# leggedrobotics/qed-splatter

Hardware: NVIDIA B200
Metric: fwd+bwd RGB+depth Mpix/s (higher is better)
Workload: dtype f32

## Files before the change

### qed_splatter_b200/csrc/isect.cu

```cuda
#include <cub/device/device_radix_sort.cuh>

#include "common.cuh"
#include "radix.cuh"
#include "scan.cuh"

namespace qed {

__global__ void isect_count_kernel(int64_t CN, const float2* __restrict__ means2d, const int32_t* __restrict__ radii,
                                   float tile_size, int tile_w, int tile_h, int32_t* __restrict__ tiles) {
    int64_t i = (int64_t)blockIdx.x * blockDim.x + threadIdx.x;
    if (i >= CN) return;
    int r = radii[i];
    int cnt = 0;
    if (r > 0) {
        float2 m = means2d[i];
        TileBox tb = tile_box(m.x, m.y, r, tile_size, tile_w, tile_h);
        cnt = (tb.x1 - tb.x0) * (tb.y1 - tb.y0);
    }
    tiles[i] = cnt;
}

__global__ void isect_emit_kernel(int C, int N, const float2* __restrict__ means2d, const int32_t* __restrict__ radii,
                                  const float* __restrict__ depths, const int64_t* __restrict__ cum, float tile_size, int tile_w,
                                  int tile_h, int tile_n_bits, int64_t* __restrict__ isect_ids, int32_t* __restrict__ flatten_ids) {
// ... 168 lines not shown
    uint64_t* tmp_keys = reinterpret_cast<uint64_t*>(ws);
    int32_t* tmp_vals = reinterpret_cast<int32_t*>(ws + align_up((size_t)n * 8, 256));
    void* hist = ws + align_up((size_t)n * 8, 256) + align_up((size_t)n * 4, 256);
    return radix_sort_pairs<uint64_t>(n, nullptr, reinterpret_cast<const uint64_t*>(keys_in), vals_in, reinterpret_cast<uint64_t*>(keys_out),
                                      vals_out, tmp_keys, tmp_vals, hist, end_bit, stream);
}

namespace qed {

struct PrepareLayout {
    size_t scan_ws, scan_state, keys[3], vals[3], hist, cum2, total;
};

static PrepareLayout prepare_layout(int64_t CN) {
    PrepareLayout L;
    size_t o = 0;
    auto take = [&](size_t bytes) {
        size_t r = o;
        o += align_up(bytes, 256);
        return r;
    };
    L.scan_ws = take(scan_workspace_bytes(CN));
    L.scan_state = take(2 * kFlatScanStateBytes);
    for (int i = 0; i < 3; ++i) L.keys[i] = take((size_t)CN * 8);
    for (int i = 0; i < 3; ++i) L.vals[i] = take((size_t)CN * 4);
    L.hist = take(radix_hist_bytes(CN));
    L.cum2 = take((size_t)CN * 8);
    L.total = o;
    return L;
}

template <typename KeyT>
struct CompactVisibleSink {
    int N;
    const float* depths;
    KeyT* keys;
    int32_t* vals;
    __device__ __forceinline__ void operator()(int64_t idx, int32_t flag, int64_t inc) const {
        if (!flag) return;
        const uint32_t db = (uint32_t)__float_as_int(depths[idx]);
        keys[inc - 1] = sizeof(KeyT) == 8 ? (KeyT)(((uint64_t)(idx / N) << 32) | db) : (KeyT)db;
        vals[inc - 1] = (int32_t)idx;
    }
};

constexpr int kEmitThreads = 256;
constexpr int kEmitTile = 1024;

__global__ void emit_boundaries_kernel(int64_t n_vis, int64_t n_isects, const int64_t* __restrict__ counts_dev, int64_t* __restrict__ clamped,
                                       const int64_t* __restrict__ cum2, int32_t* __restrict__ first_j) {
    pdl_enter();
    const int64_t j = (int64_t)blockIdx.x * blockDim.x + threadIdx.x;
    if (counts_dev) {
        const int64_t real_vis = counts_dev[0], real_isects = counts_dev[1];
        n_vis = real_vis < n_vis ? real_vis : n_vis;
        n_isects = real_isects <= n_isects ? real_isects : 0;
        if (n_isects == 0) n_vis = 0;
    }
    if (j == 0) {
        clamped[0] = n_vis;
        clamped[1] = n_isects;
    }
    if (j >= n_vis) return;
    const int64_t start = j > 0 ? cum2[j - 1] : 0, end = cum2[j];
    for (int64_t b = (start + kEmitTile - 1) / kEmitTile; b * kEmitTile < end; ++b) first_j[b] = (int32_t)j;
}

__global__ void __launch_bounds__(kEmitThreads) emit_sorted_kernel(int64_t n_vis, int64_t n_isects, const int64_t* __restrict__ clamped, int N,
                                                                  const int32_t* __restrict__ sorted_vals,
                                                                  const int64_t* __restrict__ cum2, const int32_t* __restrict__ first_j,
                                                                  const float2* __restrict__ means2d, const int32_t* __restrict__ radii,
                                                                  float tile_size, int tile_w, int tile_h, int tile_n_bits,
                                                                  uint32_t* __restrict__ tkeys, int32_t* __restrict__ tvals) {
    __shared__ int16_t s_lo[kEmitTile + 1], s_hi[kEmitTile + 1];
    __shared__ int32_t s_k0[kEmitTile + 1], s_first[kEmitTile + 1], s_idx[kEmitTile + 1];
    __shared__ int16_t s_bw[kEmitTile + 1], s_large[kEmitTile + 1];
    __shared__ __align__(16) uint32_t s_okey[kEmitTile];
    __shared__ __align__(16) int32_t s_oval[kEmitTile];
    __shared__ int s_nlarge;
    __shared__ int s_wsum[kEmitThreads / 32];
    pdl_enter();
    const uint32_t vb = blockIdx.x;
    const int64_t e0 = (int64_t)vb * kEmitTile;
    if (clamped) {
        n_vis = clamped[0];
        n_isects = clamped[1];
        if (e0 >= n_isects) return;
    }
    const int64_t e1 = min(e0 + kEmitTile, n_isects);
    const int64_t j0 = first_j[vb];
    int64_t j1;
    if (e1 >= n_isects) {
        j1 = n_vis - 1;
    } else {
        const int64_t jn = first_j[vb + 1];
        j1 = (jn > 0 && cum2[jn - 1] == e1) ? jn - 1 : jn;
// ... 27 lines not shown
            s_oval[lo + t] = idx;
            if (++rx == bw) {
                rx = 0;
                ++ry;
            }
        }
    }
    const int lane = threadIdx.x & 31, warp = threadIdx.x >> 5;
    const int nlarge = s_nlarge;
    for (int i = warp; i < nlarge; i += kEmitThreads / 32) {
        const int g = s_large[i];
        const int lo = s_lo[g], n = s_hi[g] - lo, k0 = s_k0[g];
        const int bw = s_bw[g], idx = s_idx[g], first = s_first[g];
        const float inv_bw = 1.0f / (float)bw;
        for (int t = lane; t < n; t += 32) {
            const int k = k0 + t;
            const int ry = (int)(((float)k + 0.5f) * inv_bw);
            const int rx = k - ry * bw;
            s_okey[lo + t] = (uint32_t)(first + ry * tile_w + rx);
            s_oval[lo + t] = idx;
        }
    }
    __syncthreads();
    for (int t = threadIdx.x; t < (int)(e1 - e0); t += kEmitThreads) {
        tkeys[e0 + t] = s_okey[t];
        tvals[e0 + t] = s_oval[t];
    }
}

__global__ void __launch_bounds__(kEmitThreads) emit_exact_kernel(int64_t n_vis, int64_t n_isects, const int64_t* __restrict__ clamped, int N,
                                                                 const int32_t* __restrict__ sorted_vals, const int64_t* __restrict__ cum2,
                                                                 const int32_t* __restrict__ first_j, const float2* __restrict__ means2d,
                                                                 const int32_t* __restrict__ radii, const float4* __restrict__ geom, int height,
                                                                 float tile_size, int tile_w, int tile_h, int tile_n_bits,
                                                                 uint32_t* __restrict__ tkeys, int32_t* __restrict__ tvals) {
    __shared__ int16_t s_lo[kEmitTile + 1], s_hi[kEmitTile + 1], s_large[kEmitTile + 1];
    __shared__ int32_t s_k0[kEmitTile + 1], s_idx[kEmitTile + 1];
    __shared__ __align__(16) uint32_t s_okey[kEmitTile];
    __shared__ __align__(16) int32_t s_oval[kEmitTile];
    __shared__ int s_nlarge;
    pdl_enter();
    const uint32_t vb = blockIdx.x;
    const int64_t e0 = (int64_t)vb * kEmitTile;
    if (clamped) {
        n_vis = clamped[0];
        n_isects = clamped[1];
    }
    if (e0 >= n_isects) return;
    const int64_t e1 = min(e0 + kEmitTile, n_isects);
    const int64_t j0 = first_j[vb];
    int64_t j1;
    if (e1 >= n_isects) {
        j1 = n_vis - 1;
    } else {
        const int64_t jn = first_j[vb + 1];
        j1 = (jn > 0 && cum2[jn - 1] == e1) ? jn - 1 : jn;
    }
    const int G = (int)(j1 - j0) + 1;
// ... 56 lines not shown
        const uint32_t cam_bits = (uint32_t)(idx / N) << tile_n_bits;
        int base = 0;
        for (int r0 = tb.y0; r0 < tb.y1 && base < k0 + n; r0 += 32) {
            const int ty = r0 + lane;
            int c0 = 0, c1 = 0;
            if (ty < tb.y1) exact_row_span(ec, ty, height, tb.x0, tb.x1, c0, c1);
            const int w = c1 - c0;
            int inc = w;
#pragma unroll
            for (int o = 1; o < 32; o <<= 1) {
                const int v = __shfl_up_sync(0xffffffffu, inc, o);
                if (lane >= o) inc += v;
            }
            const int row_start = base + inc - w;
            const int a = max(row_start, k0), b = min(row_start + w, k0 + n);
            for (int q = a; q < b; ++q) {
                s_okey[lo + (q - k0)] = cam_bits | (uint32_t)(ty * tile_w + c0 + (q - row_start));
                s_oval[lo + (q - k0)] = idx;
            }
            base += __shfl_sync(0xffffffffu, inc, 31);
        }
    }
    __syncthreads();
    for (int t = threadIdx.x; t < (int)(e1 - e0); t += kEmitThreads) {
        tkeys[e0 + t] = s_okey[t];
        tvals[e0 + t] = s_oval[t];
    }
}

constexpr int kComposePer = 4;
__global__ void __launch_bounds__(256) compose_ids_ranges_kernel(int64_t n_host, const int64_t* __restrict__ n_dev, const uint32_t* __restrict__ tkeys,
                                                                 const int32_t* __restrict__ flat, const float* __restrict__ depths, int C, int n_tiles,
                                                                 int tile_n_bits, int64_t* __restrict__ isect_ids, int32_t* __restrict__ offsets) {
    pdl_enter();
    const int64_t i0 = ((int64_t)blockIdx.x * blockDim.x + threadIdx.x) * kComposePer;
    const int64_t n = n_dev ? *n_dev : n_host;
    if (n_dev && offsets && i0 == 0) {
        offsets[(int64_t)C * n_tiles] = (int32_t)n;
        if (n == 0)
            for (int64_t t = 0; t < (int64_t)C * n_tiles; ++t) offsets[t] = 0;
    }
    if (i0 >= n) return;
    uint32_t key[kComposePer];
    if (i0 + kComposePer <= n) {
        const uint4 k4 = *reinterpret_cast<const uint4*>(tkeys + i0);
        key[0] = k4.x, key[1] = k4.y, key[2] = k4.z, key[3] = k4.w;
    } else {
#pragma unroll
        for (int k = 0; k < kComposePer; ++k) key[k] = i0 + k < n ? tkeys[i0 + k] : 0u;
    }
    const uint32_t mask = (1u << tile_n_bits) - 1u;
    uint32_t kp = i0 > 0 ? tkeys[i0 - 1] : 0u;
#pragma unroll
    for (int k = 0; k < kComposePer; ++k) {
        const int64_t i = i0 + k;
        if (i >= n) break;
        if (isect_ids) {
            const uint32_t db = (uint32_t)__float_as_int(depths[flat[i]]);
            isect_ids[i] = (int64_t)(((uint64_t)key[k] << 32) | db);
        }
        if (offsets) {
            const int64_t cur = (int64_t)(key[k] >> tile_n_bits) * n_tiles + (key[k] & mask);
            if (i == 0) {
                for (int64_t t = 0; t <= cur; ++t) offsets[t] = 0;
            } else if (key[k] != kp) {
                const int64_t prev = (int64_t)(kp >> tile_n_bits) * n_tiles + (kp & mask);
                for (int64_t t = prev + 1; t <= cur; ++t) offsets[t] = (int32_t)i;
            }
            if (i == n - 1) {
                for (int64_t t = cur + 1; t < (int64_t)C * n_tiles; ++t) offsets[t] = (int32_t)n;
            }
        }
        kp = key[k];
    }
}

static int bit_length(int64_t v) {
    int b = 0;
    while (((int64_t)1 << b) <= v) ++b;
    return b;
}

}

extern "C" size_t qed_isect_prepare_workspace_bytes(int64_t CN) { return prepare_layout(CN > 0 ? CN : 1).total; }

extern "C" int qed_isect_prepare(int C, int N, const float* depths, const int32_t* tiles_per_gauss, void* workspace,
                                 size_t workspace_bytes, int64_t* counts_dev, int64_t* counts_host_pinned, qed_stream_t stream_) {
    cudaStream_t stream = (cudaStream_t)stream_;
    if (C < 0 || N < 0 || !counts_dev) return QED_ERR_BAD_ARG;
    const int64_t CN = (int64_t)C * N;
    if (CN == 0) {
        QED_CUDA_TRY(cudaMemsetAsync(counts_dev, 0, 16, stream));
    } else {
        if (CN > 0x7fffffffLL) return QED_ERR_UNSUPPORTED;
        if (!depths || !tiles_per_gauss || !workspace) return QED_ERR_BAD_ARG;
        const PrepareLayout L = prepare_layout(CN);
        if (workspace_bytes < L.total) return QED_ERR_WORKSPACE;
        char* ws = reinterpret_cast<char*>(workspace);
        int32_t* vals0 = reinterpret_cast<int32_t*>(ws + L.vals[0]);
        int32_t* vals1 = reinterpret_cast<int32_t*>(ws + L.vals[1]);
        int32_t* vals2 = reinterpret_cast<int32_t*>(ws + L.vals[2]);
        int64_t* cum2 = reinterpret_cast<int64_t*>(ws + L.cum2);
        int rc;
        char* st0 = ws + L.scan_state;
        char* st1 = st0 + kFlatScanStateBytes;
        const bool flat = g_flat_scan != 0;
        if (flat) QED_CUDA_TRY(cudaMemsetAsync(st0, 0, 2 * kFlatScanStateBytes, stream));
        if (C == 1) {
            uint32_t* k0 = reinterpret_cast<uint32_t*>(ws + L.keys[0]);
            uint32_t* k1 = reinterpret_cast<uint32_t*>(ws + L.keys[1]);
            uint32_t* k2 = reinterpret_cast<uint32_t*>(ws + L.keys[2]);
            rc = flat ? scan_flat_to(CN, nullptr, ScanFlagPositive{tiles_per_gauss}, CompactVisibleSink<uint32_t>{N, depths, k0, vals0}, counts_dev, st0, stream)
                      : scan_inclusive_to(CN, nullptr, ScanFlagPositive{tiles_per_gauss}, CompactVisibleSink<uint32_t>{N, depths, k0, vals0}, counts_dev,
                                          ws + L.scan_ws, stream);
            if (rc != QED_OK) return rc;
            rc = radix_sort_pairs<uint32_t>(CN, counts_dev, k0, vals0, k1, vals1, k2, vals2, ws + L.hist, 32, stream);
        } else {
            uint64_t* k0 = reinterpret_cast<uint64_t*>(ws + L.keys[0]);
            uint64_t* k1 = reinterpret_cast<uint64_t*>(ws + L.keys[1]);
            uint64_t* k2 = reinterpret_cast<uint64_t*>(ws + L.keys[2]);
            rc = flat ? scan_flat_to(CN, nullptr, ScanFlagPositive{tiles_per_gauss}, CompactVisibleSink<uint64_t>{N, depths, k0, vals0}, counts_dev, st0, stream)
                      : scan_inclusive_to(CN, nullptr, ScanFlagPositive{tiles_per_gauss}, CompactVisibleSink<uint64_t>{N, depths, k0, vals0}, counts_dev,
                                          ws + L.scan_ws, stream);
            if (rc != QED_OK) return rc;
            rc = radix_sort_pairs<uint64_t>(CN, counts_dev, k0, vals0, k1, vals1, k2, vals2, ws + L.hist, 32 + bit_length(C - 1), stream);
        }
        if (rc != QED_OK) return rc;
        rc = flat ? scan_flat_to(CN, counts_dev, ScanGather{tiles_per_gauss, vals1}, ScanStore{cum2}, counts_dev + 1, st1, stream)
                  : scan_inclusive(CN, counts_dev, ScanGather{tiles_per_gauss, vals1}, cum2, counts_dev + 1, ws + L.scan_ws, stream);
        if (rc != QED_OK) return rc;
    }
    if (counts_host_pinned) QED_CUDA_TRY(cudaMemcpyAsync(counts_host_pinned, counts_dev, 16, cudaMemcpyDeviceToHost, stream));
    return QED_OK;
}

extern "C" size_t qed_isect_fill_workspace_bytes(int64_t n_isects) {
    if (n_isects <= 0) return 256;
    const size_t nb = (size_t)((n_isects + kEmitTile - 1) / kEmitTile + 1);
    return 5 * align_up((size_t)n_isects * 4, 256) + radix_hist_bytes(n_isects) + align_up(nb * 4, 256) + align_up(nb * 8 + 8, 256) + 256;
}

extern "C" int qed_isect_fill(int C, int N, int64_t n_visible, int64_t n_isects, const float* means2d, const int32_t* radii,
                              const float* depths, const float* geom, int image_width, int image_height, int tile_size, int tile_width,
                              int tile_height, const void* prepare_workspace, void* workspace, size_t workspace_bytes,
                              const int64_t* counts_dev, int64_t* isect_ids, int32_t* flatten_ids, int32_t* isect_offsets,
                              int64_t* n_exact_dev, qed_stream_t stream_) {
    cudaStream_t stream = (cudaStream_t)stream_;
    if (C < 0 || N < 0 || n_visible < 0 || n_isects < 0 || tile_size <= 0) return QED_ERR_BAD_ARG;
// ... 13 lines not shown
    if (n_isects > 0x7fffffffLL) return QED_ERR_UNSUPPORTED;
    if (n_exact_dev && !exact && !counts_dev && !isect_offsets) return QED_ERR_BAD_ARG;
    if (!means2d || !radii || !depths || !prepare_workspace || !workspace || !flatten_ids) return QED_ERR_BAD_ARG;
    if (workspace_bytes < qed_isect_fill_workspace_bytes(n_isects)) return QED_ERR_WORKSPACE;
    const int tile_n_bits = bit_length(n_tiles);
    const int cam_bits = bit_length(C - 1);
    if (tile_n_bits + cam_bits > 32) return QED_ERR_UNSUPPORTED;
    const PrepareLayout L = prepare_layout(CN);
    const char* pws = reinterpret_cast<const char*>(prepare_workspace);
    const int32_t* sorted_vals = reinterpret_cast<const int32_t*>(pws + L.vals[1]);
    const int64_t* cum2 = reinterpret_cast<const int64_t*>(pws + L.cum2);
    char* ws = reinterpret_cast<char*>(workspace);
    const size_t seg = align_up((size_t)n_isects * 4, 256);
    uint32_t* k0 = reinterpret_cast<uint32_t*>(ws);
    uint32_t* k1 = reinterpret_cast<uint32_t*>(ws + seg);
    uint32_t* k2 = reinterpret_cast<uint32_t*>(ws + 2 * seg);
    int32_t* v0 = reinterpret_cast<int32_t*>(ws + 3 * seg);
    int32_t* v2 = reinterpret_cast<int32_t*>(ws + 4 * seg);
    void* hist = ws + 5 * seg;
    const size_t nb = (size_t)((n_isects + kEmitTile - 1) / kEmitTile);
    int32_t* first_j = reinterpret_cast<int32_t*>(ws + 5 * seg + radix_hist_bytes(n_isects));
    int64_t* clamped = reinterpret_cast<int64_t*>(ws + 5 * seg + radix_hist_bytes(n_isects) + align_up((nb + 1) * 4, 256));
    if (n_visible == 0) return QED_ERR_BAD_ARG;
    QED_CUDA_TRY(launch_pdl(emit_boundaries_kernel, dim3((unsigned)((n_visible + 255) / 256)), dim3(256), 0, stream, n_visible, n_isects, counts_dev,
                            clamped, cum2, first_j));
    const int64_t* cl = counts_dev ? clamped : nullptr;
    if (exact) {
        QED_CUDA_TRY(launch_pdl(emit_exact_kernel, dim3((unsigned)nb), dim3(kEmitThreads), 0, stream, n_visible, n_isects, cl, N, sorted_vals, cum2,
                                first_j, reinterpret_cast<const float2*>(means2d), radii, reinterpret_cast<const float4*>(geom), image_height,
                                (float)tile_size, tile_width, tile_height, tile_n_bits, k0, v0));
    } else {
        QED_CUDA_TRY(launch_pdl(emit_sorted_kernel, dim3((unsigned)nb), dim3(kEmitThreads), 0, stream, n_visible, n_isects, cl, N, sorted_vals, cum2,
                                first_j, reinterpret_cast<const float2*>(means2d), radii, (float)tile_size, tile_width, tile_height, tile_n_bits,
                                k0, v0));
    }
    const int64_t* n_dev = has_end ? clamped + 1 : nullptr;
    int rc = radix_sort_pairs<uint32_t>(n_isects, n_dev, k0, v0, k1, flatten_ids, k2, v2, hist, tile_n_bits + cam_bits, stream);
    if (rc != QED_OK) return rc;
    QED_CUDA_TRY(launch_pdl(compose_ids_ranges_kernel, dim3((unsigned)((n_isects + 256 * kComposePer - 1) / (256 * kComposePer))), dim3(256), 0, stream,
                            n_isects, n_dev, k1, flatten_ids, depths, C, n_tiles, tile_n_bits, isect_ids, isect_offsets));
    if (n_exact_dev) QED_CUDA_TRY(cudaMemcpyAsync(n_exact_dev, clamped + 1, 8, cudaMemcpyDeviceToDevice, stream));
    return QED_OK;
}
```

### qed_splatter_b200/csrc/radix.cuh

```cuda
#pragma once
#include "common.cuh"

namespace qed {

static thread_local int g_radix_small_tiles = 0;
static thread_local int g_radix_onesweep = 1;

constexpr int kSortThreads = 256;
constexpr int kSortItems = 16;
constexpr int kSortTile = kSortThreads * kSortItems;
constexpr int kRadix = 256;

struct SegCounts {
    const int32_t* counts = nullptr;
    int shift = 0;
    __device__ __forceinline__ bool ok(int64_t i) const { return !counts || (int)(i & ((1 << shift) - 1)) < counts[i >> shift]; }
};

template <typename KeyT, bool SEG>
__global__ void __launch_bounds__(kSortThreads) radix_upsweep_kernel(int64_t n_host, const int64_t* n_dev, const KeyT* __restrict__ keys, int shift,
                                                                    uint32_t mask, int nblocks, uint32_t* __restrict__ hist , SegCounts seg) {
    __shared__ uint32_t sh[kRadix];
    pdl_enter();
    const int64_t n = n_dev ? *n_dev : n_host;
// ... 393 lines not shown
        global_base[d] = (sscan[8 + warp] + ginc - tot) + excl;
    }
    __syncthreads();
#pragma unroll
    for (int r = 0; r < kRounds; ++r) {
        const int local = warp * kPerWarp + r * 32 + lane;
        if (local < tile_n) {
            const uint32_t d = (uint32_t)(key[r] >> shift) & mask;
            const uint32_t pos = digit_start[d] + warp_hist[warp][d] + rank[r];
            skeys[pos] = key[r];
            svals[pos] = val[r];
        }
    }
    __syncthreads();
    for (int i = threadIdx.x; i < tile_n; i += kSortThreads) {
        const KeyT k = skeys[i];
        const uint32_t d = (uint32_t)(k >> shift) & mask;
        const int64_t dst = (int64_t)global_base[d] + (i - digit_start[d]);
        keys_out[dst] = k;
        vals_out[dst] = svals[i];
    }
}

inline size_t radix_hist_bytes(int64_t capacity) {
    int64_t nb = (capacity + kSortTile - 1) / kSortTile;
    if (nb < 1) nb = 1;
    return 2 * (((size_t)kRadix * nb * 4 + 255) / 256 * 256) + ((kRadix * 4 + 255) / 256 * 256) +
           (((size_t)kRadix * 2 * nb * 8 + 255) / 256 * 256) + ((size_t)(kMaxPasses * kRadix + kMaxPasses) * 4 + 255) / 256 * 256;
}

template <typename KeyT>
inline int radix_sort_pairs(int64_t capacity, const int64_t* n_dev, const KeyT* keys_in, const int32_t* vals_in, KeyT* keys_out,
                            int32_t* vals_out, KeyT* tmp_keys, int32_t* tmp_vals, void* hist_ws, int end_bit, cudaStream_t stream,
                            SegCounts seg = SegCounts()) {
    if (capacity <= 0) return QED_OK;
    const int nb = (int)((capacity + kSortTile - 1) / kSortTile);
    const size_t hist_bytes = ((size_t)kRadix * nb * 4 + 255) / 256 * 256;
    uint32_t* hist_a = reinterpret_cast<uint32_t*>(hist_ws);
    uint32_t* hist_b = reinterpret_cast<uint32_t*>(reinterpret_cast<char*>(hist_ws) + hist_bytes);
    uint32_t* totals = reinterpret_cast<uint32_t*>(reinterpret_cast<char*>(hist_ws) + 2 * hist_bytes);
    const int passes = (end_bit + 7) / 8;
    if (passes == 0) {
        if (n_dev) return QED_ERR_UNSUPPORTED;
        QED_CUDA_TRY(cudaMemcpyAsync(keys_out, keys_in, (size_t)capacity * sizeof(KeyT), cudaMemcpyDeviceToDevice, stream));
        QED_CUDA_TRY(cudaMemcpyAsync(vals_out, vals_in, (size_t)capacity * 4, cudaMemcpyDeviceToDevice, stream));
        return QED_OK;
    }
    if (!seg.counts && g_radix_onesweep && passes <= kMaxPasses && (nb <= kOnesweepMaxBlocks || g_radix_onesweep > 1)) {
        char* ows = reinterpret_cast<char*>(hist_ws) + 2 * hist_bytes + ((kRadix * 4 + 255) / 256 * 256);
        const bool small = g_radix_small_tiles && nb <= 2 * 148;
        const int nbk = small ? (int)((capacity + kSortTile / 2 - 1) / (kSortTile / 2)) : nb;
        uint64_t* status = reinterpret_cast<uint64_t*>(ows);
        const size_t status_bytes = ((size_t)kRadix * 2 * nb * 8 + 255) / 256 * 256;
        uint32_t* hist_all = reinterpret_cast<uint32_t*>(ows + status_bytes);
        uint32_t* tickets = hist_all + kMaxPasses * kRadix;
        QED_CUDA_TRY(cudaMemsetAsync(ows, 0, status_bytes + (size_t)(kMaxPasses * kRadix + kMaxPasses) * 4, stream));
        QED_CUDA_TRY(launch_pdl(radix_histogram_kernel<KeyT>, dim3(nb), dim3(kSortThreads), 0, stream, capacity, n_dev, keys_in, passes, end_bit, hist_all));
        auto one = small ? radix_onesweep_kernel<KeyT, 8> : radix_onesweep_kernel<KeyT, 16>;
        const size_t one_smem = small ? RadixSmem<KeyT>::kBytes - (size_t)(kSortTile / 2) * (sizeof(KeyT) + 4) : RadixSmem<KeyT>::kBytes;
        QED_CUDA_TRY(cudaFuncSetAttribute(one, cudaFuncAttributeMaxDynamicSharedMemorySize, (int)one_smem));
        const KeyT* sk = keys_in;
        const int32_t* sv = vals_in;
        for (int pass = 0; pass < passes; ++pass) {
            const bool to_out = ((passes - 1 - pass) % 2) == 0;
            KeyT* dk = to_out ? keys_out : tmp_keys;
            int32_t* dv = to_out ? vals_out : tmp_vals;
            const int bits = (end_bit - pass * 8) < 8 ? (end_bit - pass * 8) : 8;
            QED_CUDA_TRY(launch_pdl(one, dim3(nbk), dim3(kSortThreads), one_smem, stream, capacity, n_dev, sk, sv, dk, dv, pass * 8,
                                    (1u << bits) - 1u, pass, hist_all, status, tickets));
            sk = dk;
            sv = dv;
        }
        return QED_OK;
    }
    auto down = radix_downsweep_kernel<KeyT, false>;
    auto down_seg = radix_downsweep_kernel<KeyT, true>;
    QED_CUDA_TRY(cudaFuncSetAttribute(down, cudaFuncAttributeMaxDynamicSharedMemorySize, (int)RadixSmem<KeyT>::kBytes));
    if (seg.counts) QED_CUDA_TRY(cudaFuncSetAttribute(down_seg, cudaFuncAttributeMaxDynamicSharedMemorySize, (int)RadixSmem<KeyT>::kBytes));
    auto pass_mask = [&](int pass) {
        const int bits = (end_bit - pass * 8) < 8 ? (end_bit - pass * 8) : 8;
// ... 30 lines not shown
```

### qed_splatter_b200/csrc/scan.cuh

```cuda
#pragma once
#include "common.cuh"

namespace qed {

constexpr int kScanThreads = 256;
constexpr int kScanItems = 8;
constexpr int kScanTile = kScanThreads * kScanItems;

__device__ __forceinline__ int64_t block_exclusive_scan(int64_t v, int64_t* smem_warp, int64_t& total) {
    const int lane = threadIdx.x & 31, warp = threadIdx.x >> 5;
    int64_t inc = v;
#pragma unroll
    for (int o = 1; o < 32; o <<= 1) {
        int64_t t = __shfl_up_sync(0xffffffffu, inc, o);
        if (lane >= o) inc += t;
    }
    if (lane == 31) smem_warp[warp] = inc;
    __syncthreads();
    if (warp == 0) {
        int64_t w = lane < (kScanThreads / 32) ? smem_warp[lane] : 0;
        int64_t winc = w;
#pragma unroll
        for (int o = 1; o < 32; o <<= 1) {
            int64_t t = __shfl_up_sync(0xffffffffu, winc, o);
// ... 89 lines not shown
inline size_t scan_workspace_bytes(int64_t capacity) {
    int64_t nb = (capacity + kScanTile - 1) / kScanTile;
    return (size_t)(nb > 0 ? nb : 1) * sizeof(int64_t);
}

template <typename F, typename Sink>
inline int scan_inclusive_to(int64_t capacity, const int64_t* n_dev, F f, Sink sink, int64_t* total_dev, void* workspace, cudaStream_t stream) {
    int64_t nb = (capacity + kScanTile - 1) / kScanTile;
    if (nb == 0) nb = 1;
    int64_t* sums = reinterpret_cast<int64_t*>(workspace);
    QED_CUDA_TRY(launch_pdl(scan_reduce_kernel<F>, dim3((unsigned)nb), dim3(kScanThreads), 0, stream, capacity, n_dev, f, sums));
    QED_CUDA_TRY(launch_pdl(scan_sums_kernel, dim3(1), dim3(kScanThreads), 0, stream, nb, sums, total_dev));
    QED_CUDA_TRY(launch_pdl(scan_final_kernel<F, Sink>, dim3((unsigned)nb), dim3(kScanThreads), 0, stream, capacity, n_dev, f, sums, sink));
    return QED_OK;
}

constexpr int kFlatScanBlocks = 1024;
struct FlatScanState {
    unsigned long long agg[kFlatScanBlocks];
    unsigned int ticket, pad;
};
constexpr size_t kFlatScanStateBytes = sizeof(FlatScanState);

template <typename F, typename Sink>
__global__ void __launch_bounds__(kScanThreads) scan_flat_kernel(int64_t n_host, const int64_t* n_dev, F f, Sink sink, FlatScanState* __restrict__ st,
                                                                int64_t* __restrict__ total_dev, int tiles_per_block) {
    __shared__ int64_t sw[kScanThreads / 32 + 1];
    __shared__ unsigned int s_vb;
    pdl_enter();
    const int64_t n = n_dev ? min(*n_dev, n_host) : n_host;
    if (threadIdx.x == 0) s_vb = atomicAdd(&st->ticket, 1u);
    __syncthreads();
    const unsigned int vb = s_vb;
    const int64_t tile0 = (int64_t)vb * tiles_per_block;
    int32_t v[kScanItems];
    int64_t s = 0, ex0 = 0, total;
    if (tiles_per_block == 1) {
        const int64_t base = tile0 * kScanTile + (int64_t)threadIdx.x * kScanItems;
#pragma unroll
        for (int k = 0; k < kScanItems; ++k) {
            v[k] = (base + k < n) ? f(base + k) : 0;
            s += v[k];
        }
        ex0 = block_exclusive_scan(s, sw, total);
    } else {
        for (int t = 0; t < tiles_per_block; ++t) {
            const int64_t base = (tile0 + t) * kScanTile;
            if (base >= n) break;
#pragma unroll
            for (int k = 0; k < kScanItems; ++k) {
                const int64_t i = base + k * kScanThreads + threadIdx.x;
// ... 6 lines not shown
        volatile unsigned long long* slot = st->agg + vb;
        *slot = (1ull << 63) | (unsigned long long)total;
    }
    int64_t mine = 0;
    for (unsigned int b = threadIdx.x; b < vb; b += kScanThreads) {
        volatile const unsigned long long* slot = st->agg + b;
        unsigned long long w;
        do {
            w = *slot;
        } while (!(w >> 63));
        mine += (int64_t)(w & ~(1ull << 63));
    }
    int64_t prefix;
    block_exclusive_scan(mine, sw, prefix);
    if (vb == gridDim.x - 1 && threadIdx.x == 0 && total_dev) *total_dev = prefix + total;
    if (tiles_per_block == 1) {
        const int64_t base = tile0 * kScanTile + (int64_t)threadIdx.x * kScanItems;
        int64_t ex = ex0 + prefix;
#pragma unroll
        for (int k = 0; k < kScanItems; ++k) {
            ex += v[k];
            if (base + k < n) sink(base + k, v[k], ex);
        }
        return;
    }
    int64_t carry = prefix;
    for (int t = 0; t < tiles_per_block; ++t) {
        const int64_t tbase = (tile0 + t) * kScanTile;
        if (tbase >= n) break;
        const int64_t base = tbase + (int64_t)threadIdx.x * kScanItems;
        int64_t ts = 0;
#pragma unroll
        for (int k = 0; k < kScanItems; ++k) {
            v[k] = (base + k < n) ? f(base + k) : 0;
            ts += v[k];
        }
        int64_t tile_total;
        int64_t ex = block_exclusive_scan(ts, sw, tile_total) + carry;
#pragma unroll
        for (int k = 0; k < kScanItems; ++k) {
            ex += v[k];
            if (base + k < n) sink(base + k, v[k], ex);
        }
        carry += tile_total;
    }
}

template <typename F, typename Sink>
inline int scan_flat_to(int64_t capacity, const int64_t* n_dev, F f, Sink sink, int64_t* total_dev, void* state, cudaStream_t stream) {
    int64_t tiles = (capacity + kScanTile - 1) / kScanTile;
    if (tiles == 0) tiles = 1;
    const int blocks = (int)(tiles < kFlatScanBlocks ? tiles : kFlatScanBlocks);
    const int tiles_per_block = (int)((tiles + blocks - 1) / blocks);
    const int used = (int)((tiles + tiles_per_block - 1) / tiles_per_block);
    QED_CUDA_TRY(launch_pdl(scan_flat_kernel<F, Sink>, dim3((unsigned)used), dim3(kScanThreads), 0, stream, capacity, n_dev, f, sink,
                            reinterpret_cast<FlatScanState*>(state), total_dev, tiles_per_block));
    return QED_OK;
}

template <typename F>
inline int scan_inclusive(int64_t capacity, const int64_t* n_dev, F f, int64_t* out, int64_t* total_dev, void* workspace, cudaStream_t stream) {
    return scan_inclusive_to(capacity, n_dev, f, ScanStore{out}, total_dev, workspace, stream);
}

}
```

### qed_splatter_b200/pipeline.py

```python
from __future__ import annotations

from dataclasses import dataclass
from typing import Dict, Optional

import torch
from torch import Tensor

from . import _lib, ops
from ._lib import check, current_stream, ptr


@dataclass
class StepOutput:
    loss: Tensor
    grads: Dict[str, Tensor]
    packed_grads: Tensor
    radii: Tensor
    render: Tensor
    alphas: Tensor
    n_isects: int
    n_visible: Optional[int] = None
    v_viewmats: Optional[Tensor] = None


# ... 318 lines not shown
        def redo():
            self.overflow_repeats += 1
            return forward_and_loss(True)[2:]

        render, alphas, v_render, v_alphas = forward_and_loss(False)
        v_viewmats = self._get("v_viewmats", (C, 4, 4)) if pose_gradients else None
        grads, packed = self.backward(v_render, v_alphas, grad_out, n_chunks=n_chunks, on_chunk=on_chunk, exchange=exchange, v_viewmats=v_viewmats,
                                      _redo=redo)
        self._last_v = (v_render, v_alphas)
        f = self._fwd
        return StepOutput(loss=self._loss, grads=grads, packed_grads=packed, radii=f["radii"], render=f["render"], alphas=f["alphas"],
                          n_isects=f.get("n_isects_real", f["M"]), n_visible=f.get("n_visible"), v_viewmats=v_viewmats)

    def n_isects_exact(self) -> int:
        f = self._fwd
        return int(self._n_exact.item()) if (f.get("exact") and f["M"]) else int(f.get("n_isects_real", f["M"]))

    @property
    def launches_per_step(self) -> int:
        f = self._fwd
        tile_bits = (f["tw"] * f["th"]).bit_length()
        cam_bits = (f["C"] - 1).bit_length()

        def radix(capacity: int, bits: int, segmented: bool = False) -> int:
            passes = (bits + 7) // 8
            one_kernel_passes = (not segmented) and (capacity + 4095) // 4096 <= 444
            return 1 + passes if one_kernel_passes else 3 * passes

        if self.sort_impl == "two_level":
            isect = 1 + radix(f["C"] * f["N"], 32 + cam_bits) + 1 + 1 + 1 + radix(f["M"], tile_bits + cam_bits) + 1
        else:
            end_bit = 32 + tile_bits + f["C"].bit_length()
            isect = 3 + 1 + (radix(f["M"], end_bit) if self.sort_impl == "own" else 8) + 1
        return 1 + isect + 1 + 3 + 1 + 1

    @torch.no_grad()
    def count_pairs(self, which=("fwd", "bwd")) -> Dict[str, int]:
        lib, stream, f = self.lib, current_stream(), self._fwd
        out = {}
        if not f["M"]:
            return out
        names = ("entries_loaded", "entries_staged", "warp_candidates", "pairs_evaluated", "pairs_contributing", "reduction_groups")
        for which in which:
            cnt = torch.zeros(6, dtype=torch.int64, device=self.device)
            check(lib.qed_debug_set_raster_counters(ptr(cnt)), "set counters")
            try:
                if which == "fwd":
                    check(lib.qed_raster_fwd(f["C"], f["N"], f["M"], f["D"], ptr(f["geom"]), ptr(f["colors"]), ptr(f["backgrounds"]),
                                             f["width"], f["height"], 16, f["tw"], f["th"], ptr(f["offsets"]), int(f["has_end"]), ptr(f["flat"]),
                                             f["normalize"], ptr(f["render"]), ptr(f["alphas"]), ptr(f["last_ids"]), stream), "qed_raster_fwd(stats)")
                else:
                    v_render, v_alphas = self._last_v
                    scratch = torch.zeros(f["C"] * f["N"], 12, device=self.device)
                    check(lib.qed_raster_bwd(f["C"], f["N"], f["M"], f["D"], ptr(f["geom"]), ptr(f["colors"]), ptr(f["backgrounds"]),
                                             f["width"], f["height"], 16, f["tw"], f["th"], ptr(f["offsets"]), ptr(f["flat"]), f["normalize"],
                                             ptr(f["render"]), ptr(f["alphas"]), ptr(f["last_ids"]), ptr(v_render), ptr(v_alphas),
# ... 8 lines not shown
```

Measured before the change: 1741.

## Fuse radix histograms into producer kernels and compute tile offsets by counting

The visibility compaction scan now builds the per-pass radix digit histograms in shared memory, so the onesweep sort can skip its separate histogram kernel. The emit kernels atomically count intersections per tile bin, and a new single-block scan kernel turns those counts into tile offsets while also producing the second sort's histograms. This replaces the offset-writing logic in compose and drops the compose launch when isect ids are not requested. The memsets are merged and the workspace is reordered. In exchange it adds global and shared atomics and a serial single-block scan over all bins.

```diff
diff --git a/qed_splatter_b200/csrc/isect.cu b/qed_splatter_b200/csrc/isect.cu
--- a/qed_splatter_b200/csrc/isect.cu
+++ b/qed_splatter_b200/csrc/isect.cu
@@ -214,9 +214,9 @@
     };
     L.scan_ws = take(scan_workspace_bytes(CN));
     L.scan_state = take(2 * kFlatScanStateBytes);
+    L.hist = take(radix_hist_bytes(CN));
     for (int i = 0; i < 3; ++i) L.keys[i] = take((size_t)CN * 8);
     for (int i = 0; i < 3; ++i) L.vals[i] = take((size_t)CN * 4);
-    L.hist = take(radix_hist_bytes(CN));
     L.cum2 = take((size_t)CN * 8);
     L.total = o;
     return L;
@@ -224,15 +224,46 @@
 
 template <typename KeyT>
 struct CompactVisibleSink {
+    static constexpr int kPasses = sizeof(KeyT) == 8 ? kMaxPasses : 4;
     int N;
     const float* depths;
     KeyT* keys;
     int32_t* vals;
+    uint32_t* hist_all;
+    int end_bit;
+    __device__ static uint32_t* smem_hist() {
+        __shared__ uint32_t h[kPasses * kRadix];
+        return h;
+    }
+    __device__ __forceinline__ int passes() const { return (end_bit + 7) / 8; }
+    __device__ __forceinline__ void block_begin() const {
+        if (!hist_all) return;
+        for (int i = threadIdx.x; i < passes() * kRadix; i += blockDim.x) smem_hist()[i] = 0;
+        __syncthreads();
+    }
+    __device__ __forceinline__ void block_end() const {
+        if (!hist_all) return;
+        __syncthreads();
+        for (int i = threadIdx.x; i < passes() * kRadix; i += blockDim.x) {
+            const uint32_t c = smem_hist()[i];
+            if (c) atomicAdd(hist_all + i, c);
+        }
+    }
     __device__ __forceinline__ void operator()(int64_t idx, int32_t flag, int64_t inc) const {
         if (!flag) return;
         const uint32_t db = (uint32_t)__float_as_int(depths[idx]);
-        keys[inc - 1] = sizeof(KeyT) == 8 ? (KeyT)(((uint64_t)(idx / N) << 32) | db) : (KeyT)db;
+        const KeyT key = sizeof(KeyT) == 8 ? (KeyT)(((uint64_t)(idx / N) << 32) | db) : (KeyT)db;
+        keys[inc - 1] = key;
         vals[inc - 1] = (int32_t)idx;
+        if (hist_all) {
+            uint32_t* h = smem_hist();
+#pragma unroll
+            for (int p = 0; p < kPasses; ++p) {
+                if (p * 8 >= end_bit) break;
+                const int bits = end_bit - p * 8 < 8 ? end_bit - p * 8 : 8;
+                atomicAdd(&h[p * kRadix + ((uint32_t)(key >> (p * 8)) & ((1u << bits) - 1u))], 1u);
+            }
+        }
     }
 };
 
@@ -240,9 +271,12 @@
 constexpr int kEmitTile = 1024;
 
 __global__ void emit_boundaries_kernel(int64_t n_vis, int64_t n_isects, const int64_t* __restrict__ counts_dev, int64_t* __restrict__ clamped,
-                                       const int64_t* __restrict__ cum2, int32_t* __restrict__ first_j) {
+                                       const int64_t* __restrict__ cum2, int32_t* __restrict__ first_j, int32_t* __restrict__ bin_counts,
+                                       int64_t n_bins) {
     pdl_enter();
     const int64_t j = (int64_t)blockIdx.x * blockDim.x + threadIdx.x;
+    if (bin_counts)
+        for (int64_t t = j; t < n_bins; t += (int64_t)gridDim.x * blockDim.x) bin_counts[t] = 0;
     if (counts_dev) {
         const int64_t real_vis = counts_dev[0], real_isects = counts_dev[1];
         n_vis = real_vis < n_vis ? real_vis : n_vis;
@@ -258,12 +292,23 @@
     for (int64_t b = (start + kEmitTile - 1) / kEmitTile; b * kEmitTile < end; ++b) first_j[b] = (int32_t)j;
 }
 
+__device__ __forceinline__ void emit_store(int64_t e0, int n, const uint32_t* s_okey, const int32_t* s_oval, uint32_t* __restrict__ tkeys,
+                                           int32_t* __restrict__ tvals, int32_t* __restrict__ bin_counts, int n_tiles, int tile_n_bits) {
+    for (int t = threadIdx.x; t < n; t += kEmitThreads) {
+        const uint32_t key = s_okey[t];
+        tkeys[e0 + t] = key;
+        tvals[e0 + t] = s_oval[t];
+        if (bin_counts) atomicAdd(bin_counts + (key >> tile_n_bits) * (uint32_t)n_tiles + (key & ((1u << tile_n_bits) - 1u)), 1);
+    }
+}
+
 __global__ void __launch_bounds__(kEmitThreads) emit_sorted_kernel(int64_t n_vis, int64_t n_isects, const int64_t* __restrict__ clamped, int N,
                                                                   const int32_t* __restrict__ sorted_vals,
                                                                   const int64_t* __restrict__ cum2, const int32_t* __restrict__ first_j,
                                                                   const float2* __restrict__ means2d, const int32_t* __restrict__ radii,
                                                                   float tile_size, int tile_w, int tile_h, int tile_n_bits,
-                                                                  uint32_t* __restrict__ tkeys, int32_t* __restrict__ tvals) {
+                                                                  uint32_t* __restrict__ tkeys, int32_t* __restrict__ tvals,
+                                                                  int32_t* __restrict__ bin_counts) {
     __shared__ int16_t s_lo[kEmitTile + 1], s_hi[kEmitTile + 1];
     __shared__ int32_t s_k0[kEmitTile + 1], s_first[kEmitTile + 1], s_idx[kEmitTile + 1];
     __shared__ int16_t s_bw[kEmitTile + 1], s_large[kEmitTile + 1];
@@ -337,10 +382,7 @@
         }
     }
     __syncthreads();
-    for (int t = threadIdx.x; t < (int)(e1 - e0); t += kEmitThreads) {
-        tkeys[e0 + t] = s_okey[t];
-        tvals[e0 + t] = s_oval[t];
-    }
+    emit_store(e0, (int)(e1 - e0), s_okey, s_oval, tkeys, tvals, bin_counts, tile_w * tile_h, tile_n_bits);
 }
 
 __global__ void __launch_bounds__(kEmitThreads) emit_exact_kernel(int64_t n_vis, int64_t n_isects, const int64_t* __restrict__ clamped, int N,
@@ -348,7 +390,8 @@
                                                                  const int32_t* __restrict__ first_j, const float2* __restrict__ means2d,
                                                                  const int32_t* __restrict__ radii, const float4* __restrict__ geom, int height,
                                                                  float tile_size, int tile_w, int tile_h, int tile_n_bits,
-                                                                 uint32_t* __restrict__ tkeys, int32_t* __restrict__ tvals) {
+                                                                 uint32_t* __restrict__ tkeys, int32_t* __restrict__ tvals,
+                                                                 int32_t* __restrict__ bin_counts) {
     __shared__ int16_t s_lo[kEmitTile + 1], s_hi[kEmitTile + 1], s_large[kEmitTile + 1];
     __shared__ int32_t s_k0[kEmitTile + 1], s_idx[kEmitTile + 1];
     __shared__ __align__(16) uint32_t s_okey[kEmitTile];
@@ -451,24 +494,88 @@
         }
     }
     __syncthreads();
-    for (int t = threadIdx.x; t < (int)(e1 - e0); t += kEmitThreads) {
-        tkeys[e0 + t] = s_okey[t];
-        tvals[e0 + t] = s_oval[t];
+    emit_store(e0, (int)(e1 - e0), s_okey, s_oval, tkeys, tvals, bin_counts, tile_w * tile_h, tile_n_bits);
+}
+
+constexpr int kTileOffsetsThreads = 1024;
+constexpr int kTileOffsetsItems = 8;
+__global__ void __launch_bounds__(kTileOffsetsThreads) tile_offsets_kernel(int32_t* __restrict__ offsets, int64_t n_bins, int has_end, int n_tiles,
+                                                                          int tile_n_bits, int end_bit, uint32_t* __restrict__ hist_all,
+                                                                          int64_t* __restrict__ n_exact_dev) {
+    constexpr int kWarps = kTileOffsetsThreads / 32;
+    __shared__ uint32_t s_hist[4][kRadix];
+    __shared__ int64_t s_warp[kWarps];
+    __shared__ int64_t s_carry;
+    const int lane = threadIdx.x & 31, warp = threadIdx.x >> 5;
+    const int passes = (end_bit + 7) / 8;
+    if (hist_all)
+        for (int i = threadIdx.x; i < 4 * kRadix; i += kTileOffsetsThreads) (&s_hist[0][0])[i] = 0;
+    if (threadIdx.x == 0) s_carry = 0;
+    pdl_enter();
+    __syncthreads();
+    for (int64_t base = 0; base < n_bins; base += kTileOffsetsThreads * kTileOffsetsItems) {
+        const int64_t b0 = base + (int64_t)threadIdx.x * kTileOffsetsItems;
+        int32_t v[kTileOffsetsItems];
+        int64_t sum = 0;
+#pragma unroll
+        for (int k = 0; k < kTileOffsetsItems; ++k) {
+            v[k] = b0 + k < n_bins ? offsets[b0 + k] : 0;
+            sum += v[k];
+            if (hist_all && v[k]) {
+                const int64_t bin = b0 + k;
+                const uint32_t key = ((uint32_t)(bin / n_tiles) << tile_n_bits) | (uint32_t)(bin % n_tiles);
+                for (int p = 0; p < passes; ++p) {
+                    const int bits = end_bit - p * 8 < 8 ? end_bit - p * 8 : 8;
+                    atomicAdd(&s_hist[p][(key >> (p * 8)) & ((1u << bits) - 1u)], (uint32_t)v[k]);
+                }
+            }
+        }
+        int64_t inc = sum;
+#pragma unroll
+        for (int o = 1; o < 32; o <<= 1) {
+            const int64_t t = __shfl_up_sync(0xffffffffu, inc, o);
+            if (lane >= o) inc += t;
+        }
+        if (lane == 31) s_warp[warp] = inc;
+        __syncthreads();
+        if (warp == 0) {
+            const int64_t w = s_warp[lane];
+            int64_t winc = w;
+#pragma unroll
+            for (int o = 1; o < 32; o <<= 1) {
+                const int64_t t = __shfl_up_sync(0xffffffffu, winc, o);
+                if (lane >= o) winc += t;
+            }
+            s_warp[lane] = winc - w;
+        }
+        __syncthreads();
+        int64_t run = s_carry + s_warp[warp] + inc - sum;
+#pragma unroll
+        for (int k = 0; k < kTileOffsetsItems; ++k) {
+            if (b0 + k < n_bins) offsets[b0 + k] = (int32_t)run;
+            run += v[k];
+        }
+        __syncthreads();
+        if (threadIdx.x == kTileOffsetsThreads - 1) s_carry = run;
+        __syncthreads();
+    }
+    if (threadIdx.x == 0) {
+        if (has_end) offsets[n_bins] = (int32_t)s_carry;
+        if (n_exact_dev) *n_exact_dev = s_carry;
+    }
+    if (hist_all) {
+        __syncthreads();
+        for (int i = threadIdx.x; i < passes * kRadix; i += kTileOffsetsThreads) hist_all[i] = (&s_hist[0][0])[i];
     }
 }
 
 constexpr int kComposePer = 4;
-__global__ void __launch_bounds__(256) compose_ids_ranges_kernel(int64_t n_host, const int64_t* __restrict__ n_dev, const uint32_t* __restrict__ tkeys,
-                                                                 const int32_t* __restrict__ flat, const float* __restrict__ depths, int C, int n_tiles,
-                                                                 int tile_n_bits, int64_t* __restrict__ isect_ids, int32_t* __restrict__ offsets) {
+__global__ void __launch_bounds__(256) compose_ids_kernel(int64_t n_host, const int64_t* __restrict__ n_dev, const uint32_t* __restrict__ tkeys,
+                                                          const int32_t* __restrict__ flat, const float* __restrict__ depths,
+                                                          int64_t* __restrict__ isect_ids) {
     pdl_enter();
     const int64_t i0 = ((int64_t)blockIdx.x * blockDim.x + threadIdx.x) * kComposePer;
     const int64_t n = n_dev ? *n_dev : n_host;
-    if (n_dev && offsets && i0 == 0) {
-        offsets[(int64_t)C * n_tiles] = (int32_t)n;
-        if (n == 0)
-            for (int64_t t = 0; t < (int64_t)C * n_tiles; ++t) offsets[t] = 0;
-    }
     if (i0 >= n) return;
     uint32_t key[kComposePer];
     if (i0 + kComposePer <= n) {
@@ -478,29 +585,12 @@
 #pragma unroll
         for (int k = 0; k < kComposePer; ++k) key[k] = i0 + k < n ? tkeys[i0 + k] : 0u;
     }
-    const uint32_t mask = (1u << tile_n_bits) - 1u;
-    uint32_t kp = i0 > 0 ? tkeys[i0 - 1] : 0u;
 #pragma unroll
     for (int k = 0; k < kComposePer; ++k) {
         const int64_t i = i0 + k;
         if (i >= n) break;
-        if (isect_ids) {
-            const uint32_t db = (uint32_t)__float_as_int(depths[flat[i]]);
-            isect_ids[i] = (int64_t)(((uint64_t)key[k] << 32) | db);
-        }
-        if (offsets) {
-            const int64_t cur = (int64_t)(key[k] >> tile_n_bits) * n_tiles + (key[k] & mask);
-            if (i == 0) {
-                for (int64_t t = 0; t <= cur; ++t) offsets[t] = 0;
-            } else if (key[k] != kp) {
-                const int64_t prev = (int64_t)(kp >> tile_n_bits) * n_tiles + (kp & mask);
-                for (int64_t t = prev + 1; t <= cur; ++t) offsets[t] = (int32_t)i;
-            }
-            if (i == n - 1) {
-                for (int64_t t = cur + 1; t < (int64_t)C * n_tiles; ++t) offsets[t] = (int32_t)n;
-            }
-        }
-        kp = key[k];
+        const uint32_t db = (uint32_t)__float_as_int(depths[flat[i]]);
+        isect_ids[i] = (int64_t)(((uint64_t)key[k] << 32) | db);
     }
 }
 
@@ -535,25 +625,28 @@
         char* st0 = ws + L.scan_state;
         char* st1 = st0 + kFlatScanStateBytes;
         const bool flat = g_flat_scan != 0;
-        if (flat) QED_CUDA_TRY(cudaMemsetAsync(st0, 0, 2 * kFlatScanStateBytes, stream));
+        const int end_bit = C == 1 ? 32 : 32 + bit_length(C - 1);
+        const bool lookback = radix_lookback(CN, end_bit);
+        QED_CUDA_TRY(cudaMemsetAsync(st0, 0, (L.hist - L.scan_state) + (lookback ? radix_lookback_bytes(CN) : 0), stream));
+        uint32_t* hist_all = flat && lookback ? radix_hist_all(ws + L.hist, CN) : nullptr;
         if (C == 1) {
             uint32_t* k0 = reinterpret_cast<uint32_t*>(ws + L.keys[0]);
             uint32_t* k1 = reinterpret_cast<uint32_t*>(ws + L.keys[1]);
             uint32_t* k2 = reinterpret_cast<uint32_t*>(ws + L.keys[2]);
-            rc = flat ? scan_flat_to(CN, nullptr, ScanFlagPositive{tiles_per_gauss}, CompactVisibleSink<uint32_t>{N, depths, k0, vals0}, counts_dev, st0, stream)
-                      : scan_inclusive_to(CN, nullptr, ScanFlagPositive{tiles_per_gauss}, CompactVisibleSink<uint32_t>{N, depths, k0, vals0}, counts_dev,
-                                          ws + L.scan_ws, stream);
+            const CompactVisibleSink<uint32_t> sink{N, depths, k0, vals0, hist_all, end_bit};
+            rc = flat ? scan_flat_to(CN, nullptr, ScanFlagPositive{tiles_per_gauss}, sink, counts_dev, st0, stream)
+                      : scan_inclusive_to(CN, nullptr, ScanFlagPositive{tiles_per_gauss}, sink, counts_dev, ws + L.scan_ws, stream);
             if (rc != QED_OK) return rc;
-            rc = radix_sort_pairs<uint32_t>(CN, counts_dev, k0, vals0, k1, vals1, k2, vals2, ws + L.hist, 32, stream);
+            rc = radix_sort_pairs<uint32_t>(CN, counts_dev, k0, vals0, k1, vals1, k2, vals2, ws + L.hist, end_bit, stream, true, hist_all != nullptr);
         } else {
             uint64_t* k0 = reinterpret_cast<uint64_t*>(ws + L.keys[0]);
             uint64_t* k1 = reinterpret_cast<uint64_t*>(ws + L.keys[1]);
             uint64_t* k2 = reinterpret_cast<uint64_t*>(ws + L.keys[2]);
-            rc = flat ? scan_flat_to(CN, nullptr, ScanFlagPositive{tiles_per_gauss}, CompactVisibleSink<uint64_t>{N, depths, k0, vals0}, counts_dev, st0, stream)
-                      : scan_inclusive_to(CN, nullptr, ScanFlagPositive{tiles_per_gauss}, CompactVisibleSink<uint64_t>{N, depths, k0, vals0}, counts_dev,
-                                          ws + L.scan_ws, stream);
+            const CompactVisibleSink<uint64_t> sink{N, depths, k0, vals0, hist_all, end_bit};
+            rc = flat ? scan_flat_to(CN, nullptr, ScanFlagPositive{tiles_per_gauss}, sink, counts_dev, st0, stream)
+                      : scan_inclusive_to(CN, nullptr, ScanFlagPositive{tiles_per_gauss}, sink, counts_dev, ws + L.scan_ws, stream);
             if (rc != QED_OK) return rc;
-            rc = radix_sort_pairs<uint64_t>(CN, counts_dev, k0, vals0, k1, vals1, k2, vals2, ws + L.hist, 32 + bit_length(C - 1), stream);
+            rc = radix_sort_pairs<uint64_t>(CN, counts_dev, k0, vals0, k1, vals1, k2, vals2, ws + L.hist, end_bit, stream, true, hist_all != nullptr);
         }
         if (rc != QED_OK) return rc;
         rc = flat ? scan_flat_to(CN, counts_dev, ScanGather{tiles_per_gauss, vals1}, ScanStore{cum2}, counts_dev + 1, st1, stream)
@@ -613,23 +706,32 @@
     int32_t* first_j = reinterpret_cast<int32_t*>(ws + 5 * seg + radix_hist_bytes(n_isects));
     int64_t* clamped = reinterpret_cast<int64_t*>(ws + 5 * seg + radix_hist_bytes(n_isects) + align_up((nb + 1) * 4, 256));
     if (n_visible == 0) return QED_ERR_BAD_ARG;
+    const int64_t n_bins = (int64_t)C * n_tiles;
+    int32_t* bin_counts = isect_offsets;
+    const int end_bit = tile_n_bits + cam_bits;
+    const bool lookback = radix_lookback(n_isects, end_bit);
+    if (lookback) QED_CUDA_TRY(cudaMemsetAsync(hist, 0, radix_lookback_bytes(n_isects), stream));
     QED_CUDA_TRY(launch_pdl(emit_boundaries_kernel, dim3((unsigned)((n_visible + 255) / 256)), dim3(256), 0, stream, n_visible, n_isects, counts_dev,
-                            clamped, cum2, first_j));
+                            clamped, cum2, first_j, bin_counts, n_bins));
     const int64_t* cl = counts_dev ? clamped : nullptr;
     if (exact) {
         QED_CUDA_TRY(launch_pdl(emit_exact_kernel, dim3((unsigned)nb), dim3(kEmitThreads), 0, stream, n_visible, n_isects, cl, N, sorted_vals, cum2,
                                 first_j, reinterpret_cast<const float2*>(means2d), radii, reinterpret_cast<const float4*>(geom), image_height,
-                                (float)tile_size, tile_width, tile_height, tile_n_bits, k0, v0));
+                                (float)tile_size, tile_width, tile_height, tile_n_bits, k0, v0, bin_counts));
     } else {
         QED_CUDA_TRY(launch_pdl(emit_sorted_kernel, dim3((unsigned)nb), dim3(kEmitThreads), 0, stream, n_visible, n_isects, cl, N, sorted_vals, cum2,
                                 first_j, reinterpret_cast<const float2*>(means2d), radii, (float)tile_size, tile_width, tile_height, tile_n_bits,
-                                k0, v0));
+                                k0, v0, bin_counts));
     }
     const int64_t* n_dev = has_end ? clamped + 1 : nullptr;
-    int rc = radix_sort_pairs<uint32_t>(n_isects, n_dev, k0, v0, k1, flatten_ids, k2, v2, hist, tile_n_bits + cam_bits, stream);
+    uint32_t* hist_all = bin_counts && lookback ? radix_hist_all(hist, n_isects) : nullptr;
+    if (bin_counts)
+        QED_CUDA_TRY(launch_pdl(tile_offsets_kernel, dim3(1), dim3(kTileOffsetsThreads), 0, stream, bin_counts, n_bins, (int)has_end, n_tiles,
+                                tile_n_bits, end_bit, hist_all, n_exact_dev));
+    int rc = radix_sort_pairs<uint32_t>(n_isects, n_dev, k0, v0, k1, flatten_ids, k2, v2, hist, end_bit, stream, lookback, hist_all != nullptr);
     if (rc != QED_OK) return rc;
-    QED_CUDA_TRY(launch_pdl(compose_ids_ranges_kernel, dim3((unsigned)((n_isects + 256 * kComposePer - 1) / (256 * kComposePer))), dim3(256), 0, stream,
-                            n_isects, n_dev, k1, flatten_ids, depths, C, n_tiles, tile_n_bits, isect_ids, isect_offsets));
-    if (n_exact_dev) QED_CUDA_TRY(cudaMemcpyAsync(n_exact_dev, clamped + 1, 8, cudaMemcpyDeviceToDevice, stream));
+    if (isect_ids)
+        QED_CUDA_TRY(launch_pdl(compose_ids_kernel, dim3((unsigned)((n_isects + 256 * kComposePer - 1) / (256 * kComposePer))), dim3(256), 0, stream,
+                                n_isects, n_dev, k1, flatten_ids, depths, isect_ids));
     return QED_OK;
 }
diff --git a/qed_splatter_b200/csrc/radix.cuh b/qed_splatter_b200/csrc/radix.cuh
--- a/qed_splatter_b200/csrc/radix.cuh
+++ b/qed_splatter_b200/csrc/radix.cuh
@@ -439,23 +439,34 @@
     }
 }
 
+inline int64_t radix_blocks(int64_t capacity) { return capacity > kSortTile ? (capacity + kSortTile - 1) / kSortTile : 1; }
+inline size_t radix_status_bytes(int64_t capacity) { return ((size_t)kRadix * 2 * radix_blocks(capacity) * 8 + 255) / 256 * 256; }
+inline size_t radix_lookback_bytes(int64_t capacity) {
+    return radix_status_bytes(capacity) + ((size_t)(kMaxPasses * kRadix + kMaxPasses) * 4 + 255) / 256 * 256;
+}
+inline uint32_t* radix_hist_all(void* hist_ws, int64_t capacity) {
+    return reinterpret_cast<uint32_t*>(reinterpret_cast<char*>(hist_ws) + radix_status_bytes(capacity));
+}
 inline size_t radix_hist_bytes(int64_t capacity) {
-    int64_t nb = (capacity + kSortTile - 1) / kSortTile;
-    if (nb < 1) nb = 1;
-    return 2 * (((size_t)kRadix * nb * 4 + 255) / 256 * 256) + ((kRadix * 4 + 255) / 256 * 256) +
-           (((size_t)kRadix * 2 * nb * 8 + 255) / 256 * 256) + ((size_t)(kMaxPasses * kRadix + kMaxPasses) * 4 + 255) / 256 * 256;
+    return radix_lookback_bytes(capacity) + 2 * (((size_t)kRadix * radix_blocks(capacity) * 4 + 255) / 256 * 256) + ((kRadix * 4 + 255) / 256 * 256);
+}
+
+inline bool radix_lookback(int64_t capacity, int end_bit) {
+    const int passes = (end_bit + 7) / 8;
+    return g_radix_onesweep && passes > 0 && passes <= kMaxPasses && (radix_blocks(capacity) <= kOnesweepMaxBlocks || g_radix_onesweep > 1);
 }
 
 template <typename KeyT>
 inline int radix_sort_pairs(int64_t capacity, const int64_t* n_dev, const KeyT* keys_in, const int32_t* vals_in, KeyT* keys_out,
                             int32_t* vals_out, KeyT* tmp_keys, int32_t* tmp_vals, void* hist_ws, int end_bit, cudaStream_t stream,
-                            SegCounts seg = SegCounts()) {
+                            bool state_zeroed = false, bool hist_ready = false, SegCounts seg = SegCounts()) {
     if (capacity <= 0) return QED_OK;
-    const int nb = (int)((capacity + kSortTile - 1) / kSortTile);
+    const int nb = (int)radix_blocks(capacity);
     const size_t hist_bytes = ((size_t)kRadix * nb * 4 + 255) / 256 * 256;
-    uint32_t* hist_a = reinterpret_cast<uint32_t*>(hist_ws);
-    uint32_t* hist_b = reinterpret_cast<uint32_t*>(reinterpret_cast<char*>(hist_ws) + hist_bytes);
-    uint32_t* totals = reinterpret_cast<uint32_t*>(reinterpret_cast<char*>(hist_ws) + 2 * hist_bytes);
+    char* three = reinterpret_cast<char*>(hist_ws) + radix_lookback_bytes(capacity);
+    uint32_t* hist_a = reinterpret_cast<uint32_t*>(three);
+    uint32_t* hist_b = reinterpret_cast<uint32_t*>(three + hist_bytes);
+    uint32_t* totals = reinterpret_cast<uint32_t*>(three + 2 * hist_bytes);
     const int passes = (end_bit + 7) / 8;
     if (passes == 0) {
         if (n_dev) return QED_ERR_UNSUPPORTED;
@@ -463,16 +474,15 @@
         QED_CUDA_TRY(cudaMemcpyAsync(vals_out, vals_in, (size_t)capacity * 4, cudaMemcpyDeviceToDevice, stream));
         return QED_OK;
     }
-    if (!seg.counts && g_radix_onesweep && passes <= kMaxPasses && (nb <= kOnesweepMaxBlocks || g_radix_onesweep > 1)) {
-        char* ows = reinterpret_cast<char*>(hist_ws) + 2 * hist_bytes + ((kRadix * 4 + 255) / 256 * 256);
+    if (!seg.counts && radix_lookback(capacity, end_bit)) {
         const bool small = g_radix_small_tiles && nb <= 2 * 148;
         const int nbk = small ? (int)((capacity + kSortTile / 2 - 1) / (kSortTile / 2)) : nb;
-        uint64_t* status = reinterpret_cast<uint64_t*>(ows);
-        const size_t status_bytes = ((size_t)kRadix * 2 * nb * 8 + 255) / 256 * 256;
-        uint32_t* hist_all = reinterpret_cast<uint32_t*>(ows + status_bytes);
+        uint64_t* status = reinterpret_cast<uint64_t*>(hist_ws);
+        uint32_t* hist_all = radix_hist_all(hist_ws, capacity);
         uint32_t* tickets = hist_all + kMaxPasses * kRadix;
-        QED_CUDA_TRY(cudaMemsetAsync(ows, 0, status_bytes + (size_t)(kMaxPasses * kRadix + kMaxPasses) * 4, stream));
-        QED_CUDA_TRY(launch_pdl(radix_histogram_kernel<KeyT>, dim3(nb), dim3(kSortThreads), 0, stream, capacity, n_dev, keys_in, passes, end_bit, hist_all));
+        if (!state_zeroed) QED_CUDA_TRY(cudaMemsetAsync(hist_ws, 0, radix_lookback_bytes(capacity), stream));
+        if (!hist_ready)
+            QED_CUDA_TRY(launch_pdl(radix_histogram_kernel<KeyT>, dim3(nb), dim3(kSortThreads), 0, stream, capacity, n_dev, keys_in, passes, end_bit, hist_all));
         auto one = small ? radix_onesweep_kernel<KeyT, 8> : radix_onesweep_kernel<KeyT, 16>;
         const size_t one_smem = small ? RadixSmem<KeyT>::kBytes - (size_t)(kSortTile / 2) * (sizeof(KeyT) + 4) : RadixSmem<KeyT>::kBytes;
         QED_CUDA_TRY(cudaFuncSetAttribute(one, cudaFuncAttributeMaxDynamicSharedMemorySize, (int)one_smem));
diff --git a/qed_splatter_b200/csrc/scan.cuh b/qed_splatter_b200/csrc/scan.cuh
--- a/qed_splatter_b200/csrc/scan.cuh
+++ b/qed_splatter_b200/csrc/scan.cuh
@@ -1,4 +1,6 @@
 #pragma once
+#include <type_traits>
+
 #include "common.cuh"
 
 namespace qed {
@@ -135,11 +137,17 @@
 };
 constexpr size_t kFlatScanStateBytes = sizeof(FlatScanState);
 
+template <typename S, typename = void>
+struct SinkHasBlockHooks : std::false_type {};
+template <typename S>
+struct SinkHasBlockHooks<S, std::void_t<decltype(&S::block_end)>> : std::true_type {};
+
 template <typename F, typename Sink>
 __global__ void __launch_bounds__(kScanThreads) scan_flat_kernel(int64_t n_host, const int64_t* n_dev, F f, Sink sink, FlatScanState* __restrict__ st,
                                                                 int64_t* __restrict__ total_dev, int tiles_per_block) {
     __shared__ int64_t sw[kScanThreads / 32 + 1];
     __shared__ unsigned int s_vb;
+    if constexpr (SinkHasBlockHooks<Sink>::value) sink.block_begin();
     pdl_enter();
     const int64_t n = n_dev ? min(*n_dev, n_host) : n_host;
     if (threadIdx.x == 0) s_vb = atomicAdd(&st->ticket, 1u);
@@ -192,6 +200,7 @@
             ex += v[k];
             if (base + k < n) sink(base + k, v[k], ex);
         }
+        if constexpr (SinkHasBlockHooks<Sink>::value) sink.block_end();
         return;
     }
     int64_t carry = prefix;
@@ -214,6 +223,7 @@
         }
         carry += tile_total;
     }
+    if constexpr (SinkHasBlockHooks<Sink>::value) sink.block_end();
 }
 
 template <typename F, typename Sink>
diff --git a/qed_splatter_b200/pipeline.py b/qed_splatter_b200/pipeline.py
--- a/qed_splatter_b200/pipeline.py
+++ b/qed_splatter_b200/pipeline.py
@@ -364,16 +364,18 @@
         tile_bits = (f["tw"] * f["th"]).bit_length()
         cam_bits = (f["C"] - 1).bit_length()
 
-        def radix(capacity: int, bits: int, segmented: bool = False) -> int:
+        def radix(capacity: int, bits: int, counted: bool) -> int:
             passes = (bits + 7) // 8
-            one_kernel_passes = (not segmented) and (capacity + 4095) // 4096 <= 444
-            return 1 + passes if one_kernel_passes else 3 * passes
+            if (capacity + 4095) // 4096 <= 444:
+                return passes + (0 if counted else 1)
+            return 3 * passes
 
         if self.sort_impl == "two_level":
-            isect = 1 + radix(f["C"] * f["N"], 32 + cam_bits) + 1 + 1 + 1 + radix(f["M"], tile_bits + cam_bits) + 1
+            isect = (1 + radix(f["C"] * f["N"], 32 + cam_bits, True) + 1 + 1 + 1 + 1 + radix(f["M"], tile_bits + cam_bits, True)
+                     + int(self.want_isect_ids))
         else:
             end_bit = 32 + tile_bits + f["C"].bit_length()
-            isect = 3 + 1 + (radix(f["M"], end_bit) if self.sort_impl == "own" else 8) + 1
+            isect = 3 + 1 + (radix(f["M"], end_bit, False) if self.sort_impl == "own" else 8) + 1
         return 1 + isect + 1 + 3 + 1 + 1
 
     @torch.no_grad()
```

New measurement: 1705, median of 6. -2.1%, worse.
